# ziatdinovmax/pyroVED

Hardware: AMD Instinct MI355X
Metric: images/sec (SVI step) (higher is better)
Workload: dtype bf16; 1 GPU; C2 iVAE 28x28 invariances=['r','t'] latent_dim=2 bernoulli, batch 256 per GPU (global 256), bf16 MFMA operands for the hidden-layer contractions (fp32 accumulate; fp32 elsewhere); the guide (fc encoder, sample, split) runs in the decoder launch's prologue in fp32, SVI step = ELBO+grads+Adam; parallelism=dp1

## Files before the change

include/pyroved_amd.h:

```cpp
#ifndef PYROVED_AMD_H
#define PYROVED_AMD_H

#include <stdint.h>

#ifdef __cplusplus
extern "C" {
#endif

#define PV_ABI_VERSION 17

#define PV_EINVAL   (-1)
#define PV_EWS      (-2)
#define PV_ECOLL    (-3)

enum pv_act {
  PV_ACT_NONE = 0, PV_ACT_TANH = 1, PV_ACT_RELU = 2, PV_ACT_LRELU = 3,
  PV_ACT_SOFTPLUS = 4, PV_ACT_GELU = 5, PV_ACT_SIGMOID = 6
};

enum pv_lik { PV_LIK_BERNOULLI = 0, PV_LIK_GAUSSIAN = 1, PV_LIK_CBERNOULLI = 2 ,
  PV_LIK_POISSON_LOG = 3 };

enum pv_kl_mode { PV_KL_SAMPLED = 0, PV_KL_ANALYTIC = 1 };

// ... 87 lines not shown
  float   lr, adam_beta1, adam_beta2, adam_eps;
  int32_t adam_step;
  int32_t flags;
  void*   ev_start;
  void*   ev_stop;
  const float* class_onehot;
  void*   conv_ev_start;
  void*   conv_ev_stop;
  double* conv_ev_flops;
  int32_t dec_kernel;
  int32_t kl_mode;
} pv_ivae_plan;

int pv_version(void);
int pv_experiments_build(void);

#define PV_PLAN_ENC_TWO_LAUNCH 1
#define PV_PLAN_NO_SIDE_STREAM 2
#define PV_PLAN_ENC_NO_WAIT    4
#define PV_PLAN_NO_DEC1D       8
#define PV_PLAN_NO_ENC_FOLD    16
#define PV_PLAN_ENC_TILED      32
#define PV_PLAN_CONV_X3        64

int64_t pv_ivae_workspace_bytes(const pv_ivae_plan* plan);
#define PV_WS_ALL    0
#define PV_WS_STEP   1
#define PV_WS_ENCODE 2
#define PV_WS_DECODE 3
int64_t pv_ivae_workspace_bytes_for(const pv_ivae_plan* plan, int what);

int pv_ivae_uses_fused(const pv_ivae_plan* plan);

int pv_ivae_guide_folds(const pv_ivae_plan* plan);

int pv_ivae_loss_and_grads(const pv_ivae_plan* plan, int want_grads, void* stream);

int pv_adam_step(float* params, float* grads, float* m, float* v, int64_t n,
                 float lr, float beta1, float beta2, float eps, int32_t step, void* stream);

int pv_adam_step_hist(float* params, float* grads, float* m, float* v, int64_t n,
                      float lr, float beta1, float beta2, float eps, int32_t step,
                      const float* scalars_src, float* scalars_dst, int32_t n_scalars, void* stream);

int pv_ivae_guide(const pv_ivae_plan* plan, void* stream);
int pv_ivae_guide_backward(const pv_ivae_plan* plan, int want_grads, void* stream);
// ... 138 lines not shown
```

pyroved_amd/_abi.py:

```python
import contextlib
import ctypes as C
import functools
import os
import threading

import torch

PV_ABI_VERSION = 17
PV_PLAN_ENC_TWO_LAUNCH, PV_PLAN_NO_SIDE_STREAM, PV_PLAN_ENC_NO_WAIT, PV_PLAN_NO_DEC1D, PV_PLAN_NO_ENC_FOLD = 1, 2, 4, 8, 16
PV_PLAN_CONV_X3 = 64
PV_PLAN_ENC_TILED = 32
PV_MAX_LAYERS = 8

ACT = {None: 0, "none": 0, "tanh": 1, "relu": 2, "lrelu": 3, "softplus": 4, "gelu": 5, "sigmoid": 6}
LIK = {"bernoulli": 0, "gaussian": 1, "continuous_bernoulli": 2, "poisson_log": 3}
KL = {"sampled": 0, "analytic": 1}

_HERE = os.path.dirname(os.path.abspath(__file__))
LIB_PATH = os.environ.get("PV_LIB_PATH") or os.path.join(_HERE, "libpyroved_amd.so")
EXP_LIB_PATH = os.path.join(_HERE, "libpyroved_amd_exp.so")

c_float_p = C.POINTER(C.c_float)


class pv_layer(C.Structure):
    _fields_ = [("in_dim", C.c_int32), ("out_dim", C.c_int32), ("act", C.c_int32), ("_pad", C.c_int32),
                ("w_off", C.c_int64), ("b_off", C.c_int64)]


PV_MAX_OPS = 32
OP = {"conv": 1, "maxpool2": 2, "upsample2": 3, "upsample2_bilinear": 4, "batchnorm": 5}


class pv_op(C.Structure):
# ... 218 lines not shown
```

pyroved_amd/csrc/pv_plan.hip:

```cpp
#include "pv_common.h"
#include <algorithm>
#include <cmath>
#include <stdlib.h>
#include "pv_kernels.h"
#include "pv_sdec_fused.h"
#include "pv_linear.h"
#include "pv_convstack.h"
#include "pv_side.h"
#include "pv_conv.h"
#include "pv_particles.h"

namespace {

struct Carver {
  char* base;
  int64_t off;
  float* take(int64_t nfloats) {
    float* p = base ? (float*)(base + off) : nullptr;
    off += pv_align_up(nfloats * (int64_t)sizeof(float), 256);
    return p;
  }
};

struct Layout {
// ... 803 lines not shown
    if (L.renyi) pb.ll_s = L.llkb;
    if (st.chain) {
      pb.enc_n = p->n_enc; pb.enc_params = p->params; pb.enc_head = p->head;
      for (int i = 0; i < p->n_enc; ++i) { pb.enc_l[i] = p->enc[i]; pb.enc_act[i] = L.eact[i]; pb.enc_dp[i] = L.edp[i]; }
    }
  }
  st.wz = wgrad_problem(L.dhz, H, st.zin, st.ldz, p->grads + p->fc_latent.w_off, p->grads + p->fc_coord.b_off, S, lat_in, H);
  if (st.chain && f.part_rs && f.dhz_out && f.dzc_out && K == 0 && !p->row_w && p->kl_mode == PV_KL_SAMPLED && !p->row_elbo &&
      !p->dy && p->head.out_dim <= 16 && p->n_enc == 2 && p->enc[0].out_dim == FD_H && p->enc[1].in_dim == FD_H &&
      p->enc[1].out_dim == FD_H && p->head.in_dim == FD_H) {
    st.tail_np = one_launch_wgrad_problems(p, L, &st.wz, 1, st.tail);
    if (st.tail_np > 0 && adam) {
      auto lsz = [](const pv_layer& l) { return (int64_t)l.in_dim * l.out_dim + (l.b_off >= 0 ? l.out_dim : 0); };
      int64_t want = lsz(p->head) + lsz(p->fc_coord) + lsz(p->fc_latent) + lsz(p->out);
      for (int i = 0; i < p->n_enc; ++i) want += lsz(p->enc[i]);
      for (int i = 0; i < p->n_dec; ++i) want += lsz(p->dec[i]);
      int64_t cov = 2 * (int64_t)H * H + (int64_t)H * (3 + p->coord_dim) + 1;
      for (int i = 0; i < st.tail_np; ++i) cov += (int64_t)st.tail[i].M * st.tail[i].N + (st.tail[i].rowsumA ? st.tail[i].M : 0);
      if (cov != want || !adam_done || p->n_dec != 2) st.tail_np = -1;
    }
  }
  if (st.own_chain()) {
    PvEncFold& ef = st.ef;
    ef.chain = 1; ef.dhead = L.dhead; ef.ldh = (int)plan_head_w(p); ef.edp0 = L.edp[0]; ef.edp1 = L.edp[1]; ef.llb = L.llb;
  }
}

int fused_decoder_launch(FusedStep& st) {
  const pv_ivae_plan* p = st.p;
  const bool timed = p->ev_start && p->ev_stop;
  if (timed) (void)hipEventRecord((hipEvent_t)p->ev_start, st.s);
  if (p->fused >= 2) PV_TRY(pv_sdec_fused_bf16_launch(st.f, st.L.f_grid, st.grads, p->fused == 2, st.s, st.fold ? &st.ef : nullptr,
                                                      (st.own_chain() && !st.fold) ? &st.ef : nullptr));
  else PV_TRY(pv_sdec_fused_launch(st.f, st.L.f_grid, st.grads, st.s));
  if (timed) (void)hipEventRecord((hipEvent_t)p->ev_stop, st.s);
  return 0;
}

int fused_close_forward(const FusedStep& st) {
  const pv_ivae_plan* p = st.p; const Layout& L = st.L; hipStream_t s = st.s;
  const int64_t B = p->batch, N = p->n_pix, K = plan_K(p);
  if (K > 0) {
    PvLatentBwd lf{};
    lf.llrow = L.llrow; lf.llb = L.llb; lf.M = L.rows; lf.N = (int)N; lf.H = 0; lf.K = (int)K; lf.alpha = L.alpha;
    lf.hb.B = (int)B; lf.fwd_only = 1;
    PV_TRY(pv_latent_bwd(lf, s));
    return pv_finish_scalars(L.llb, (int)B, p->scalars, L.kl_part, L.kl_blocks, 1.0f, s);
// ... 552 lines not shown
```

pyroved_amd/csrc/pv_sdec_fused.h:

```cpp
#pragma once
#include "pv_common.h"

#define FD_H 128
#define FD_UNIT 16
#define FD_WAVES 8
#define FD_REC (2 * FD_H * FD_H + 14 * FD_H)
#define PV_RS_W 8
#define FB_WIMG_BYTES (4 * FD_H * FD_H * 2 + 256)

struct PvFused {
  const float* x;
  const float* grid;
  const float* tp;
  const float* hz;
  float hz_scale;
  const float *Wc, *bc;
  const float *W1, *b1;
  const float *W2, *b2;
  const float *wo, *bo;
  float* llrow;
  float* loc;
  float* rowtp;
  float* part_hz;
  float* part_rs;
// ... 10 lines not shown
  int64_t units;
  int N, cd, B, lik, sigmoid_out, kmax;
  int ablate;
  int qswap;
  float sig;
  int sel;
  int dl_exp;
};

struct PvEncFold {
  const float* params;
  pv_layer enc0, enc1, head;
  const float* x; int64_t ldx;
  const float* eps;
  float* eact0; float* eact1;
  float* head_out;
  float* z; float* z_scale; float* z_loc_out; float* z_scale_out;
  float* tp;
  float* kl_part;
  float* hz; const float* Wz;
  int lat_in, z_dim, coord_dim, has_r, has_t, has_s;
  float tp0, tp1, sc_prior, beta;
  int img_per_wg;
  int chain;
  float* dhead; int ldh;
  float* edp0; float* edp1;
  float* llb;
  int coop;
  unsigned* coop_flags;
};
#if defined(__HIP_DEVICE_COMPILE__)
typedef const __attribute__((address_space(4))) PvEncFold* PvEncFoldArg;
__device__ __forceinline__ PvEncFoldArg pv_kernarg_fold() {
  const __attribute__((address_space(4))) char* k = (const __attribute__((address_space(4))) char*)__builtin_amdgcn_kernarg_segment_ptr();
  PvEncFoldArg p = (PvEncFoldArg)(k + ((sizeof(PvFused) + alignof(PvEncFold) - 1) / alignof(PvEncFold)) * alignof(PvEncFold));
  asm volatile("" : "+s"(p));
  return p;
}
#else
typedef const PvEncFold* PvEncFoldArg;
__device__ inline PvEncFoldArg pv_kernarg_fold() { return nullptr; }
#endif
#define PV_GUIDE_IMG_MAX_BATCH 384
struct PvFbPrep;
bool pv_guide_img_ok(const PvEncFold& e, int B);
int pv_guide_img_launch(const PvEncFold& e, const PvFbPrep* prep, float hz_mul, int B, hipStream_t s, int kl_mode = PV_KL_SAMPLED);
// ... 152 lines not shown
```

pyroved_amd/csrc/pv_sdec_fused_w8.hip:

```cpp
#include "pv_sdec_fused.h"
#include "pv_fb_layout.h"
#include "pv_sdec_prims.h"
#include "pv_kernels.h"
#include <stdlib.h>

#define W8_WAVES 8
#define W8_ROWS (W8_WAVES * FD_UNIT)
#define W8_THREADS (64 * W8_WAVES)
#define W8_ARR (W8_ROWS * LDS2)
#define W8_ARR_BYTES (2 * W8_ARR)
#define WO_W1 0
#define WO_W2 IMG_BYTES
#define WO_SA (2 * IMG_BYTES)
#define WO_SB (WO_SA + W8_ARR_BYTES)
#define WO_VEC (WO_SB + W8_ARR_BYTES)
#define WO_ATAB (WO_VEC + 3 * FD_H * 4)
#define WO_TTAB (WO_ATAB + 8 * 64 * 8)
#define WO_INFO (WO_TTAB + 4 * 64 * 16)
#define WO_RED (WO_INFO + 3 * W8_ROWS * 4)
#define WO_CHZ (WO_RED + 256)
#define WO_CTP (WO_CHZ + W8_WAVES * FD_H * 4)
#define WO_CGR (WO_CTP + W8_WAVES * 256)
#define W8_LDS_BYTES (WO_CGR + W8_WAVES * 256)
#define WO_TX (WO_SB + 2 * 32 * LDS2)
// ... 6 lines not shown
#ifndef W8_FENCE_MASK
#define W8_FENCE_MASK 0
#endif
#define W8_FENCE() __builtin_amdgcn_sched_barrier(W8_FENCE_MASK)

__device__ __forceinline__ float w8_tanhc(float cx) {
  const float e = __builtin_amdgcn_exp2f(cx);
  return 1.0f - 2.0f * __builtin_amdgcn_rcpf(e + 1.0f);
}
#ifndef W8_HSWAP
#define W8_HSWAP 0
#endif
#ifndef W8_QSWAP
#define W8_QSWAP 1
#endif
bool pv_sdec_fused_w8_qswap() { return W8_QSWAP != 0; }
__device__ __forceinline__ bf16x8 w8_catq(const bf16x4& a, const bf16x4& b, int q) {
  return W8_QSWAP ? sd_catq(a, b, q >= 2) : sd_cat(a, b);
}
__device__ __forceinline__ float w8_sum_q(float v) {
  return pv_sum_rows(v);
}

#ifndef W8_ABL
#define W8_ABL 0
#endif
#ifndef W8_TAIL
#define W8_TAIL 1
#endif
#ifndef W8_OWN_SUMS
#define W8_OWN_SUMS 1
#endif
#define W8_ABL_LOADS(bit, g) (!(W8_ABL & (bit)) || (((g) & 1) == 0))
#define W8_ABL_BUF(bit, g) ((W8_ABL & (bit)) ? (((g) >> 1) & 1) : ((g) & 1))


struct W8Addr : SdAddr { int fs, hs; };
__device__ __forceinline__ W8Addr w8_addr(int r, int q) {
  W8Addr a;
  a.fs = W8_HSWAP ? ((r >> 2) & 1) : 0;
  a.hs = W8_HSWAP ? (q & 1) : (W8_QSWAP ? ((r >> 1) & 1) : 0);
  static_cast<SdAddr&>(a) = sd_addr(r, q);
  return a;
}

__device__ __forceinline__ void w8_layer_fwd(const __bf16* __restrict__ Wh, const float* __restrict__ bs,
// ... 103 lines not shown
#endif
  for (int ks = 0; ks < ksteps; ++ks) {
#if W8_ABL & 4
    if ((ks & 1) == 0) {
#else
    bf16x8 a[2], b[4];
    {
#endif
    a[0] = sd_cat(sd_tr_at(la0), sd_tr_at(la0 + ROW16));
    a[1] = sd_cat(sd_tr_at(la1), sd_tr_at(la1 + ROW16));
#pragma unroll
    for (int o = 0; o < 4; ++o) b[o] = sd_cat(sd_tr_at(lb + 32u * o), sd_tr_at(lb + 32u * o + ROW16));
    }
    W8_FENCE();
    accB = MFMA32(a[0], ones, accB);
#pragma unroll
    for (int o = 0; o < 4; ++o)
#pragma unroll
      for (int s_ = 0; s_ < 2; ++s_) accW[s_][o] = MFMA32(a[s_], b[o], accW[s_][o]);
    W8_FENCE();
    la0 += 2 * ROW16; la1 += 2 * ROW16; lb += 2 * ROW16;
  }
}

__device__ __forceinline__ void w8_colsum_mfma(__bf16* __restrict__ sc, const bf16x4 (&t)[8], const bf16x4& bop,
                                               f32x4 (&accS)[8], int wave, int r, int q) {
  sd_stage_store(sc, t, 16 * wave + r, q);
  sd_wait_lgkm0();
  const __bf16* base = sc + (16 * wave) * LDS2 + sd_stage_toff(r | sd_opaque0(), q);
  bf16x4 a[8];
#pragma unroll
  for (int jb = 0; jb < 8; ++jb) a[jb] = sd_tr(base + 16 * jb);
#pragma unroll
  for (int jb = 0; jb < 8; ++jb) accS[jb] = sd_mfma16(a[jb], bop, accS[jb]);
}

#ifdef W8_TRACE
__device__ long long w8_trace[512];
#define W8_STAMP(k)                                                                              \
  do {                                                                                           \
    if (g == 0 && lane == 0 && (wave == 0 || wave == 7) && tile_no < 8)                          \
      w8_trace[(wave ? 256 : 0) + tile_no * 16 + (k)] = (long long)__builtin_readcyclecounter(); \
  } while (0)
extern "C" int pv_debug_read_trace_w8(long long* out, int n) {
  if (n > 512) n = 512;
  return (int)hipMemcpyFromSymbol(out, HIP_SYMBOL(w8_trace), n * sizeof(long long));
// ... 62 lines not shown
  for (int i = 0; i < 4; ++i) h[i] = (__bf16)v[i];
  return h;
}
__device__ __forceinline__ f32x4 w8_mul_dtanh4(const f32x4& d, const bf16x4& hb) {
  const f32x4 t = sd_f32_of(hb);
  return d * (t * t - 1.0f);
}

#define WF_H1 WO_SA
#define WF_H2 (WF_H1 + 512)
#define WF_HD (WF_H2 + 512)
#define WF_P (WF_HD + 512)
#define WF_P_WAVE (64 * 17 * 4)
static_assert(WF_P + W8_WAVES * WF_P_WAVE <= WO_VEC, "guide scratch fits in the staging arrays");
#include "pv_gemv16.h"

#define W8_COOP_SPINS 4096
__device__ unsigned w8_coop_late_total;
extern "C" int pv_debug_coop_late_count(unsigned* out) {
  return (int)hipMemcpyFromSymbol(out, HIP_SYMBOL(w8_coop_late_total), sizeof(unsigned));
}
template <bool GRADS, int LIK, int FOLDK>
__global__ __launch_bounds__(W8_THREADS) void pv_sdec_w8_kernel(PvFused f, PvEncFold e) {
  constexpr bool FOLD = FOLDK != 0, CHAIN = FOLDK >= 2, COOP = FOLDK == 3;
  constexpr bool OWN = W8_OWN_SUMS && CHAIN && GRADS;
  extern __shared__ __attribute__((aligned(16))) char smb[];
  const int tid = threadIdx.x, lane0 = tid & 63, lane = lane0, r = lane & 15, q = lane >> 4;
  const int wave = __builtin_amdgcn_readfirstlane(tid >> 6);
  const int g = blockIdx.x, G = gridDim.x;
  const unsigned lds0 = __builtin_amdgcn_readfirstlane((unsigned)(size_t)smb);
  const __bf16* W1h = reinterpret_cast<const __bf16*>(smb + WO_W1);
  const __bf16* W2h = reinterpret_cast<const __bf16*>(smb + WO_W2);
  __bf16* sA = reinterpret_cast<__bf16*>(smb + WO_SA);
  __bf16* sB = reinterpret_cast<__bf16*>(smb + WO_SB);
  float* vec = reinterpret_cast<float*>(smb + WO_VEC);
  float* info = reinterpret_cast<float*>(smb + WO_INFO);
  float* red = reinterpret_cast<float*>(smb + WO_RED);
  const char* gimg = reinterpret_cast<const char*>(f.wimg);
  W8_STAMP_K(0);
  f32x4 xr[4], xpk;
  f32x4 xc[4][4];
  unsigned coop_tag = 0;
  if (COOP) {
    coop_tag = e.coop_flags[G] + 1u;
    const int K4 = (int)(e.ldx >> 2);
#pragma unroll
    for (int i = 0; i < 4; ++i) {
// ... 289 lines not shown
    __bf16* i1 = reinterpret_cast<__bf16*>(smb + WO_W1);
    __bf16* i2 = reinterpret_cast<__bf16*>(smb + WO_W2);
#pragma unroll
    for (int u = 0; u < 8; ++u) {
      const int idx = tid + W8_THREADS * u, row = idx >> 5, c4 = idx & 31;
      us4 h1, h2;
#pragma unroll
      for (int i = 0; i < 4; ++i) {
        h1[i] = __builtin_bit_cast(unsigned short, (__bf16)(w1v[u][i] * SD_C));
        h2[i] = __builtin_bit_cast(unsigned short, (__bf16)(w2v[u][i] * SD_C));
      }
      const int el = fb_wel(row, fb_pcol(4 * c4)) ^ (W8_HSWAP ? 4 * ((row >> 2) & 1) : 0) ^ (W8_QSWAP ? 4 * ((c4 >> 1) & 1) : 0);
      *reinterpret_cast<us4*>(i1 + el) = h1;
      *reinterpret_cast<us4*>(i2 + el) = h2;
    }
  }
  sd_wait_vm0();
  __syncthreads();
  W8_STAMP_K(1);
  const float bo = f.bo[0];
  typedef __attribute__((address_space(1))) float gfloat;
  unsigned long long u_llrow = 0, u_loc, u_rowtp = 0, u_part_hz = 0;
  int64_t a_M = 0;
  if constexpr (OWN) {
    asm volatile("s_mov_b64 %0, %1" : "=&s"(u_loc) : "s"((unsigned long long)f.loc));
  } else {
    asm volatile("s_mov_b64 %0, %5\n\ts_mov_b64 %1, %6\n\ts_mov_b64 %2, %7\n\ts_mov_b64 %3, %8\n\ts_mov_b64 %4, %9"
                 : "=&s"(u_llrow), "=&s"(u_loc), "=&s"(u_rowtp), "=&s"(u_part_hz), "=&s"(a_M)
                 : "s"((unsigned long long)f.llrow), "s"((unsigned long long)f.loc), "s"((unsigned long long)f.rowtp),
                   "s"((unsigned long long)f.part_hz), "s"(f.M));
  }
  gfloat* a_llrow = (gfloat*)u_llrow; gfloat* a_loc = (gfloat*)u_loc; gfloat* a_rowtp = (gfloat*)u_rowtp;
  gfloat* a_part_hz = (gfloat*)u_part_hz;

  f32x4 accW1[2][4], accW2[2][4], accS[8], accB1 = {0, 0, 0, 0}, accB2 = {0, 0, 0, 0};
#pragma unroll
  for (int kb = 0; kb < 8; ++kb) {
    accW1[kb >> 2][kb & 3] = f32x4{0, 0, 0, 0}; accW2[kb >> 2][kb & 3] = f32x4{0, 0, 0, 0}; accS[kb] = f32x4{0, 0, 0, 0};
  }
  float dbo = 0.0f;
  float llacc = 0.0f;
  int cur_b = -1;
  const int upb = f.N / FD_UNIT;
  float* rec = f.part + (int64_t)g * FD_REC;

  auto flush_hz = [&](int b) {
    const int64_t ub = (int64_t)b * upb;
    const int gfirst = (int)(((ub + 1) * G + f.units - 1) / f.units) - 1;
    gfloat* dst = a_part_hz + ((int64_t)b * f.kmax + (g - gfirst) * W8_WAVES + wave) * FD_H + 4 * q;
    if (r == 0) {
#pragma unroll
      for (int jb = 0; jb < 8; ++jb) *(__attribute__((address_space(1))) f32x4*)(dst + 16 * jb) = accS[jb] * SD_RC2;
    }
#pragma unroll
    for (int jb = 0; jb < 8; ++jb)
#pragma unroll
      for (int i = 0; i < 4; ++i) accS[jb][i] = r == 0 ? 0.0f : accS[jb][i];
  };

  const int u_lo = (int)((int64_t)g * f.units / G), u_hi = (int)((int64_t)(g + 1) * f.units / G);
  const int xun = (int)f.x_units;
  struct Pos { int unit, b, loc, xu; };
  auto pos_of = [&](int unit_) {
    Pos p_;
    p_.unit = unit_; p_.b = unit_ / upb; p_.loc = unit_ - p_.b * upb; p_.xu = xun > 0 ? unit_ % xun : unit_;
    return p_;
  };
  auto advance = [&](Pos& p_, int by) {
    p_.unit += by; p_.loc += by; p_.xu += by;
    while (p_.loc >= upb) { p_.loc -= upb; ++p_.b; }
    if (xun > 0) { while (p_.xu >= xun) p_.xu -= xun; }
  };
  const bool has_tail = W8_TAIL && ((u_hi - u_lo) & (W8_WAVES - 1)) == 1;
  const int u_end = has_tail ? u_hi - 1 : u_hi;
  const Pos pos_lo = pos_of(has_tail ? u_end : u_lo);
  Pos pos_cur = pos_of(u_lo + wave < u_end ? u_lo + wave : (has_tail ? u_end : u_lo));
  Pos pos_nx = pos_cur;
  float sw_next = 1.0f;
  auto x_of = [&](const Pos& p_) -> float {
    if (f.sw) sw_next = f.sw[p_.b];
    return f.x[(int64_t)p_.xu * FD_UNIT + r];
  };
  float xv_next = x_of(pos_cur);
  float* chz = reinterpret_cast<float*>(smb + WO_CHZ) + wave * FD_H;
  float* ctp = reinterpret_cast<float*>(smb + WO_CTP) + wave * 64;
  float* cgr = reinterpret_cast<float*>(smb + WO_CGR) + wave * 64;
  auto fetch_unit_inputs = [&](const Pos& p_, bool first) {
    const int n0 = p_.loc * FD_UNIT;
    if (!OWN || first) {
      sd_glds4(f.hz + (int64_t)p_.b * FD_H + lane, lds0 + WO_CHZ + wave * (FD_H * 4));
      sd_glds4(f.hz + (int64_t)p_.b * FD_H + 64 + lane, lds0 + WO_CHZ + wave * (FD_H * 4) + 256);
      sd_glds4(f.tp + (int64_t)p_.b * 8 + (lane & 7), lds0 + WO_CTP + wave * 256);
    }
    sd_glds4(f.grid + (int64_t)n0 * f.cd + (lane & (16 * f.cd - 1)), lds0 + WO_CGR + wave * 256);
  };
  fetch_unit_inputs(pos_cur, true);
  const W8Addr wad = w8_addr(r, q);
  int tile_no = -1;
  for (int ut = u_lo; ut < u_end; ut += W8_WAVES) {
    ++tile_no;
    (void)tile_no;
    asm volatile("; W8_TILE_BEGIN");
    W8_STAMP(0);
    const int nact = (u_end - ut) < W8_WAVES ? (u_end - ut) : W8_WAVES;
    if (ut + W8_WAVES + wave < u_end) advance(pos_nx, W8_WAVES);
    else pos_nx = pos_lo;
    int opq = 0;
    asm volatile("" : "+v"(opq));
    const int lane = lane0 | opq, r = lane & 15, q = lane >> 4;
    const float* wos = vec;
    const float* b1s = vec + FD_H;
    const float* b2s = vec + 2 * FD_H;
    const bool act = wave < nact;
    const int unit = act ? pos_cur.unit : ut;
    const int bu = pos_cur.b;
    const int64_t row = (int64_t)unit * FD_UNIT + r;
    float x0, x1, u0c, u1c, sc;
    sd_wait_vm0();
    {
      const float* t = ctp;
      const float* gr = cgr;
      if (f.cd == 2) {
        const float gx = gr[2 * r], gy = gr[2 * r + 1];
        u0c = gx * t[0] - gy * t[1];
        u1c = gx * t[1] + gy * t[0];
        sc = t[2];
        x0 = u0c * sc + t[3];
        x1 = u1c * sc + t[4];
      } else {
        u0c = gr[r]; u1c = 0.0f; sc = 1.0f;
        x0 = u0c + t[3]; x1 = 0.0f;
      }
    }
    const float xv = xv_next, swv = sw_next;
    float* inf_x0 = info + 16 * wave;
    float* inf_x1 = info + W8_ROWS + 16 * wave;
    float* inf_dl = info + 2 * W8_ROWS + 16 * wave;

    f32x4 tC[8];
    bf16x4 pA[8], h0b[8], h1b[8];
    float dlda = 0.0f;
    {
      bf16x4 bx = sd_zero4();
      {
        const float v = q == 0 ? x0 : x1;
        __bf16 vh, vl;
        fb_split(v, vh, vl);
        const __bf16 one = (__bf16)1.0f;
        if (q < 2) { bx[0] = vh; bx[1] = vl; bx[2] = vh; }
        else if (q == 2) { bx[0] = one; bx[1] = one; }
      }
      const bf16x4* atab = reinterpret_cast<const bf16x4*>(smb + WO_ATAB) + lane;
      const float* hzb = chz;
      bf16x4 aop[8];
#pragma unroll
      for (int jb = 0; jb < 8; ++jb) {
        tC[jb] = *reinterpret_cast<const f32x4*>(hzb + 16 * jb + 4 * q);
        aop[jb] = atab[64 * jb];
      }
      if (GRADS && q == 0) { inf_x0[r] = x0; inf_x1[r] = x1; }
      W8_FENCE();
      if (f.hz_scale == 0.0f) {
#pragma unroll
        for (int jb = 0; jb < 8; ++jb) tC[jb] = tC[jb] * SD_C;
      }
      W8_FENCE();
#pragma unroll
      for (int jb = 0; jb < 8; ++jb) tC[jb] = sd_mfma16(aop[jb], bx, tC[jb]);
      W8_FENCE();
      sd_tanh8<W8_FENCE_MASK>(tC);
      w8_cvt8(tC, h0b);
    }
    asm volatile("; W8_P1_coord_done");
    W8_STAMP(1);
    fetch_unit_inputs(pos_nx, false);
    {
      w8_layer_fwd(W1h, b1s, h0b, tC, wad, q);
      sd_tanh8<W8_FENCE_MASK>(tC);
      w8_cvt8(tC, h1b);
      asm volatile("; W8_P2_l1_done");
    W8_STAMP(2);
      w8_layer_fwd(W2h, b2s, h1b, tC, wad, q);
      sd_tanh8<W8_FENCE_MASK>(tC);
      f32x4 part4 = {0.0f, 0.0f, 0.0f, 0.0f};
#pragma unroll
      for (int jb = 0; jb < 8; ++jb) {
        const f32x4 wv = *reinterpret_cast<const f32x4*>(wos + 16 * jb + 4 * q);
        part4 = part4 + tC[jb] * wv;
        if (GRADS) {
#pragma unroll
          for (int i = 0; i < 4; ++i) pA[jb][i] = (__bf16)tC[jb][i];
          const f32x4 t2 = tC[jb] * tC[jb];
          tC[jb] = wv - wv * t2;
        }
      }
      const float a = w8_sum_q((part4[0] + part4[1]) + (part4[2] + part4[3])) + bo;
      float ll, locv;
      sd_pixel_lik<LIK>(a, xv, f.sig, f.sigmoid_out, ll, dlda, locv);
      dlda *= act ? swv : 0.0f;
      if (q == 0) {
        if (act) {
          if constexpr (OWN) llacc += ll;
          else if (a_llrow) a_llrow[row] = ll;
          if (a_loc) a_loc[row] = locv;
        }
        if (GRADS) { dbo += dlda; inf_dl[r] = dlda; }
      }
      xv_next = x_of(pos_nx);
    }
    pos_cur = pos_nx;
    asm volatile("; W8_P3_fwd_done");
    W8_STAMP(3);
    if (!GRADS) continue;
    const int ksteps = (nact + 1) >> 1;
    {
      sd_wait_lgkm0();
      const f32x4 d4 = *reinterpret_cast<const f32x4*>(inf_dl + 4 * q);
      bf16x4 bw = sd_zero4();
#pragma unroll
      for (int i = 0; i < 4; ++i) {
        __bf16 hi, lo;
        fb_split(d4[i], hi, lo);
        bw[i] = r == 3 ? hi : (r == 4 ? lo : (__bf16)0.0f);
      }
      w8_colsum_mfma(sA, pA, bw, accS, wave, r, q);
#pragma unroll
      for (int jb = 0; jb < 8; ++jb) tC[jb] = tC[jb] * dlda;
      w8_cvt8(tC, pA);
    }
    asm volatile("; W8_P4_dwo_done");
    W8_STAMP(4);
    sd_stage_store(sA, pA, 16 * wave + r, q);
    sd_stage_store(sB, h1b, 16 * wave + r, q);
    __syncthreads();
    asm volatile("; W8_P5_bar1");
    W8_STAMP(5);
    w8_wgrad_consume(sA, sB, accW2, accB2, wave, r, q, ksteps);
    asm volatile("; W8_P6_cons2");
    W8_STAMP(6);
    bf16x4 p0[8];
    {
      w8_layer_dgrad(W2h, pA, tC, wad);
      w8_mul_dtanh(tC, h1b);
      w8_cvt8(tC, pA);
      asm volatile("; W8_P7_dgrad2");
    W8_STAMP(7);
      w8_layer_dgrad(W1h, pA, tC, wad);
      w8_mul_dtanh(tC, h0b);
      w8_cvt8(tC, p0);
    }
    asm volatile("; W8_P8_dgrad1");
    W8_STAMP(8);
    __syncthreads();
    W8_STAMP(9);
    {
      if constexpr (!OWN) {
        f32x4 dd = {0.0f, 0.0f, 0.0f, 0.0f};
        const bf16x8* ttab = reinterpret_cast<const bf16x8*>(smb + WO_TTAB) + lane;
#pragma unroll
        for (int mm = 0; mm < 4; ++mm) dd = MFMA32(ttab[64 * mm], sd_cat(p0[2 * mm], p0[2 * mm + 1]), dd);
// ... 2 lines not shown
          a_rowtp[row] = sc * (d1 * u0c - d0 * u1c);
          a_rowtp[a_M + row] = d0 * u0c + d1 * u1c;
          a_rowtp[2 * a_M + row] = d0;
          a_rowtp[3 * a_M + row] = d1;
        }
        if (act && bu != cur_b) {
          if (cur_b >= 0) flush_hz(cur_b);
          cur_b = bu;
        }
      }
      const f32x4 a0 = *reinterpret_cast<const f32x4*>(inf_x0 + 4 * q);
      const f32x4 a1 = *reinterpret_cast<const f32x4*>(inf_x1 + 4 * q);
      bf16x4 bc_ = sd_zero4();
      const bool use1 = r == 2 || r == 6, lo_col = r >= 5;
#pragma unroll
      for (int i = 0; i < 4; ++i) {
        __bf16 hi, lo;
        fb_split(use1 ? a1[i] : a0[i], hi, lo);
        __bf16 v = lo_col ? lo : hi;
        if (r == 0) v = (__bf16)1.0f;
        if (r == 3 || r == 4 || r > 6) v = (__bf16)0.0f;
        bc_[i] = v;
      }
      w8_colsum_mfma(sA, p0, bc_, accS, wave, r, q);
      sd_wait_lgkm0();
    }
    asm volatile("; W8_P12_rowlocal");
    W8_STAMP(12);
    sd_stage_store(sA, pA, 16 * wave + r, q);
    sd_stage_store(sB, h0b, 16 * wave + r, q);
    __syncthreads();
    asm volatile("; W8_P10_bar3");
    W8_STAMP(10);
    w8_wgrad_consume(sA, sB, accW1, accB1, wave, r, q, ksteps);
    asm volatile("; W8_P11_cons1");
    W8_STAMP(11);
    __syncthreads();
    asm volatile("; W8_P13_bar4");
    W8_STAMP(13);
    W8_STAMP(14);
    asm volatile("; W8_TILE_END");
  }

  if (has_tail) {
    asm volatile("; W8_TAIL_BEGIN");
    const int lane = lane0, r = lane & 15, q = lane >> 4;
    const float* wos = vec;
    const float* b1s = vec + FD_H;
    const float* b2s = vec + 2 * FD_H;
    const int unit = u_end, bu = pos_cur.b;
    const int64_t row = (int64_t)unit * FD_UNIT + r;
    float x0, x1, u0c, u1c, sc;
    sd_wait_vm0();
    {
      const float* t = ctp;
      const float* gr = cgr;
      if (f.cd == 2) {
        const float gx = gr[2 * r], gy = gr[2 * r + 1];
        u0c = gx * t[0] - gy * t[1];
        u1c = gx * t[1] + gy * t[0];
        sc = t[2];
        x0 = u0c * sc + t[3];
        x1 = u1c * sc + t[4];
      } else {
        u0c = gr[r]; u1c = 0.0f; sc = 1.0f;
        x0 = u0c + t[3]; x1 = 0.0f;
      }
    }
    const float xv = xv_next, swv = sw_next;
// ... 417 lines not shown
      if (tid < FD_H) {
        float y = 0.0f;
#pragma unroll
        for (int jg = 0; jg < 16; ++jg) y += cs[256 + 128 * jg + tid];
        y *= pv_act_grad2(ch_a0, 0.0f, ep_->enc0.act);
        ep_->edp0[(int64_t)g * FD_H + tid] = y;
      }
    }
  }
  if (tid == 0) {
    float v = 0.0f;
    for (int w = 0; w < W8_WAVES; ++w) v += red[w];
    rec[2 * FD_H * FD_H + 5 * FD_H] = v;
  }
  W8_STAMP_K(3);
}

bool pv_sdec_fused_w8_fold_ok(const PvFused& f, int grid) {
  if (f.N % FD_UNIT != 0 || f.N > 1024 || f.N % 4 != 0 || grid < 1 || f.B % grid != 0 || f.x_units != 0) return false;
  const int ipw = f.B / grid;
  return ipw == 1 && f.units == (int64_t)f.B * (f.N / FD_UNIT);
}

int pv_sdec_fused_w8_launch(const PvFused& f_in, int grid, bool grads, hipStream_t s, const PvEncFold* fold) {
  PvFused f = f_in;
  static const int ablate = pv_exp_int("PV_FD_ABLATE", 0) & 1024;
  f.ablate = ablate;
  const size_t lds = W8_LDS_BYTES;
  const void* fn = nullptr;
  PvEncFold e{};
  if (fold) {
    if (!pv_sdec_fused_w8_fold_ok(f, grid)) return PV_EINVAL;
    e = *fold;
    e.img_per_wg = f.B / grid;
    if (e.coop && !(grid == 256 && e.enc0.out_dim == FD_H && e.coop_flags && e.chain)) e.coop = 0;
#ifndef PV_EXPERIMENTS
    e.coop = 0;
#endif
  }
#ifdef PV_EXPERIMENTS
#define W8_COOP_BUILD 3
#else
#define W8_COOP_BUILD 2
#endif
  const bool chain = fold && e.chain;
  if (chain && grads && !(f.part_rs && f.dhz_out && f.dzc_out)) return PV_EINVAL;
#define W8_PICK(G, L) fn = !fold ? reinterpret_cast<const void*>(&pv_sdec_w8_kernel<G, L, 0>)                     \
                               : (G && chain && e.coop) ? reinterpret_cast<const void*>(&pv_sdec_w8_kernel<G, L, G ? W8_COOP_BUILD : 1>) \
                               : (G && chain) ? reinterpret_cast<const void*>(&pv_sdec_w8_kernel<G, L, G ? 2 : 1>) \
                                                : reinterpret_cast<const void*>(&pv_sdec_w8_kernel<G, L, 1>)
  if (grads) {
    if (f.lik == PV_LIK_BERNOULLI) W8_PICK(true, PV_LIK_BERNOULLI);
    else if (f.lik == PV_LIK_GAUSSIAN) W8_PICK(true, PV_LIK_GAUSSIAN);
    else if (f.lik == PV_LIK_POISSON_LOG) W8_PICK(true, PV_LIK_POISSON_LOG);
    else W8_PICK(true, PV_LIK_CBERNOULLI);
  } else {
    if (f.lik == PV_LIK_BERNOULLI) W8_PICK(false, PV_LIK_BERNOULLI);
    else if (f.lik == PV_LIK_GAUSSIAN) W8_PICK(false, PV_LIK_GAUSSIAN);
    else if (f.lik == PV_LIK_POISSON_LOG) W8_PICK(false, PV_LIK_POISSON_LOG);
    else W8_PICK(false, PV_LIK_CBERNOULLI);
  }
#undef W8_PICK
  PV_TRY(pv_set_dynamic_lds(fn, (int)lds));
  void* args[] = {&f, &e};
  hipError_t e2 = hipLaunchKernel(fn, dim3(grid), dim3(W8_THREADS), args, lds, s);
  if (e2 != hipSuccess) return (int)e2;
  PV_LAUNCH_CHECK();
  return 0;
}
```

pyroved_amd/engine.py:

```python
import ctypes as C
import math
from typing import Dict, List, Optional

import torch
import torch.nn as nn

from . import _abi
from .nets.fc import fcEncoderNet, jfcEncoderNet, fcDecoderNet, sDecoderNet
from .nets.conv import convEncoderNet
from ._convplan import UnsupportedModel, conv_ops, fill_ops, bn_modules

ALIGN = 64
N_SCALARS = 4


def _kl_name(kl) -> str:
    if kl not in _abi.KL:
        raise ValueError("kl must be 'sampled' or 'analytic' (got %r)" % (kl,))
    return kl


def _particle_count(p) -> int:
    if isinstance(p, bool) or not isinstance(p, int) or p < 1:
        raise ValueError("particles must be an int >= 1 (got %r)" % (p,))
# ... 8 lines not shown
    a = float(a)
    if not math.isfinite(a) or a == 1.0:
        raise ValueError("renyi: alpha must be a finite float other than 1 (got %r); alpha -> 1 is the multi-particle ELBO, "
                         "which particles=P without renyi computes" % (a,))
    return a


def _linears(seq: nn.Sequential) -> List[nn.Linear]:
    return [m for m in seq if isinstance(m, nn.Linear)]


class IVAEEngine:
    supports_dp_step = True
    supports_scalars_out = True
    supports_step = True
    dec_kernel = 0
    enc_two_launch = False
    enc_no_wait = False
    side_stream = True
    dec1d = True
    enc_per_image = True
    conv_x3 = False
    enc_fold = True
    kl = "sampled"
    renyi = None

    def __init__(self, model, lr: float = 1e-3, betas=(0.9, 0.999), eps: float = 1e-8, fused: int = 2, kl: str = "sampled",
                 particles: int = 1, renyi=None):
        self.model = model
        self.kl = _kl_name(kl)
        self.particles = _particle_count(particles)
        self.renyi = _renyi_alpha(renyi)
        self.lr, self.betas, self.adam_eps = float(lr), (float(betas[0]), float(betas[1])), float(eps)
        self.fused = int(fused)
        self.adam_t = 0
        self.grads_live = False
        self.device = None
        self.flat = self.grad = self.m = self.v = None
        self.ws = None
        self.events = (None, None)
        self._bn_enc, self._bn_dec = [], []
        self._enc_opt = None
        self._enc_params = []
        self._layout: Dict[str, int] = {}
        self._views: Dict[str, torch.Tensor] = {}
        self._check_model()
# ... 274 lines not shown
        if not self._conv_slices or self.wide_weights:
            return
        self._conv_tick += 1
        if not force and self._conv_tick % self._CONV_W_EVERY != 1:
            return
        if torch.cuda.is_current_stream_capturing():
            self._conv_tick -= 1
            return
        mx = float(torch.stack([self.flat[o:o + n].abs().max() for o, n in self._conv_slices]).max())
        if mx >= self._CONV_W_HI or 0.0 < mx < self._CONV_W_LO or mx != mx:
            import warnings
            warnings.warn("pyroved_amd: a convolution weight reached |w| = %.3g, outside the range of the fp16-piece "
                          "kernels; this model switches to the range-free bf16-piece convolution kernels (three pieces at "
                          "fp32-class precision, the two-piece mixed form at the throughput precision)" % mx)
            self.wide_weights = True

    def _plan_flags(self) -> int:
        return ((_abi.PV_PLAN_ENC_TWO_LAUNCH if getattr(self, "enc_two_launch", False) else 0) |
                (0 if getattr(self, "side_stream", True) else _abi.PV_PLAN_NO_SIDE_STREAM) |
                (_abi.PV_PLAN_ENC_NO_WAIT if getattr(self, "enc_no_wait", False) else 0) |
                (0 if getattr(self, "dec1d", True) else _abi.PV_PLAN_NO_DEC1D) |
                (0 if getattr(self, "enc_fold", True) else _abi.PV_PLAN_NO_ENC_FOLD) |
                (0 if getattr(self, "enc_per_image", True) else _abi.PV_PLAN_ENC_TILED) |
                (_abi.PV_PLAN_CONV_X3 if getattr(self, "conv_x3", False) else 0))

    def ensure_bound(self):
        if not self._bound():
            self.bind()

    def _layer(self, prefix: str, lin: nn.Linear, act) -> _abi.pv_layer:
        l = _abi.pv_layer()
        l.in_dim, l.out_dim, l.act = lin.in_features, lin.out_features, _abi.ACT[act]
        l.w_off = self._layout[prefix + ".weight"]
        l.b_off = self._layout[prefix + ".bias"] if lin.bias is not None else -1
        return l

    def _fc_encoder_plan(self, p, enc, m):
        idx = [i for i, mod in enumerate(enc.fc_layers) if isinstance(mod, nn.Linear)]
        p.n_enc = len(idx)
        for j, i in enumerate(idx):
            p.enc[j] = self._layer("encoder_z.fc_layers.%d" % i, enc.fc_layers[i], enc.activation)
        h = _abi.pv_layer()
        h.in_dim, h.out_dim, h.act = enc.fc11.in_features, 2 * m.z_dim + self.K, 0
        h.w_off, h.b_off = self._layout["encoder_z.fc11.weight"], self._layout["encoder_z.fc11.bias"]
        assert self._layout["encoder_z.fc12.weight"] == h.w_off + enc.fc11.weight.numel()
        assert self._layout["encoder_z.fc12.bias"] == h.b_off + enc.fc11.bias.numel()
# ... 405 lines not shown
```

Before: 2.781 million images/s.

## Add specialized full-tile decoder loop for image-owning fused training kernel

Adds a FOLDK==4 template build of the fused w8 decoder kernel used when each workgroup owns one image whose unit count is a multiple of the wave count (plus an optional tail). Applicable configurations are ones with no sample weights, 2-D coordinates, a nonzero hz scale and a non-Gaussian likelihood. This build drops per-tile position bookkeeping, partial-tile masking and runtime branches, and uses compile-time-unrolled weight-gradient consumes. It also prefetches the grid straight into LDS with global_load_lds and precomputes the staging offsets once per tile. The cost is another kernel instantiation (more code and compile time), and a plan flag is added to fall back to the generic loop.

```diff
diff --git a/include/pyroved_amd.h b/include/pyroved_amd.h
--- a/include/pyroved_amd.h
+++ b/include/pyroved_amd.h
@@ -133,6 +133,7 @@
 #define PV_PLAN_NO_ENC_FOLD    16
 #define PV_PLAN_ENC_TILED      32
 #define PV_PLAN_CONV_X3        64
+#define PV_PLAN_GENERIC_TILE_LOOP 128
 
 int64_t pv_ivae_workspace_bytes(const pv_ivae_plan* plan);
 #define PV_WS_ALL    0
diff --git a/pyroved_amd/_abi.py b/pyroved_amd/_abi.py
--- a/pyroved_amd/_abi.py
+++ b/pyroved_amd/_abi.py
@@ -10,6 +10,7 @@
 PV_PLAN_ENC_TWO_LAUNCH, PV_PLAN_NO_SIDE_STREAM, PV_PLAN_ENC_NO_WAIT, PV_PLAN_NO_DEC1D, PV_PLAN_NO_ENC_FOLD = 1, 2, 4, 8, 16
 PV_PLAN_CONV_X3 = 64
 PV_PLAN_ENC_TILED = 32
+PV_PLAN_GENERIC_TILE_LOOP = 128
 PV_MAX_LAYERS = 8
 
 ACT = {None: 0, "none": 0, "tanh": 1, "relu": 2, "lrelu": 3, "softplus": 4, "gelu": 5, "sigmoid": 6}
diff --git a/pyroved_amd/csrc/pv_plan.hip b/pyroved_amd/csrc/pv_plan.hip
--- a/pyroved_amd/csrc/pv_plan.hip
+++ b/pyroved_amd/csrc/pv_plan.hip
@@ -849,7 +849,8 @@
   }
   if (st.own_chain()) {
     PvEncFold& ef = st.ef;
-    ef.chain = 1; ef.dhead = L.dhead; ef.ldh = (int)plan_head_w(p); ef.edp0 = L.edp[0]; ef.edp1 = L.edp[1]; ef.llb = L.llb;
+    ef.chain = 1 | ((p->flags & PV_PLAN_GENERIC_TILE_LOOP) ? PV_CHAIN_GENERIC_LOOP : 0);
+    ef.dhead = L.dhead; ef.ldh = (int)plan_head_w(p); ef.edp0 = L.edp[0]; ef.edp1 = L.edp[1]; ef.llb = L.llb;
   }
 }
 
diff --git a/pyroved_amd/csrc/pv_sdec_fused.h b/pyroved_amd/csrc/pv_sdec_fused.h
--- a/pyroved_amd/csrc/pv_sdec_fused.h
+++ b/pyroved_amd/csrc/pv_sdec_fused.h
@@ -56,6 +56,7 @@
   int lat_in, z_dim, coord_dim, has_r, has_t, has_s;
   float tp0, tp1, sc_prior, beta;
   int img_per_wg;
+#define PV_CHAIN_GENERIC_LOOP 2
   int chain;
   float* dhead; int ldh;
   float* edp0; float* edp1;
diff --git a/pyroved_amd/csrc/pv_sdec_fused_w8.hip b/pyroved_amd/csrc/pv_sdec_fused_w8.hip
--- a/pyroved_amd/csrc/pv_sdec_fused_w8.hip
+++ b/pyroved_amd/csrc/pv_sdec_fused_w8.hip
@@ -52,6 +52,12 @@
   return pv_sum_rows(v);
 }
 
+__device__ __forceinline__ void w8_glds4_s(const __attribute__((address_space(1))) void* sbase, unsigned voff, unsigned lds_dst) {
+  unsigned keep;
+  asm volatile("s_mov_b32 %0, m0\n\ts_mov_b32 m0, %3\n\ts_nop 0\n\tglobal_load_lds_dword %1, %2\n\ts_mov_b32 m0, %0"
+               : "=&s"(keep) : "v"(voff), "s"(sbase), "s"(lds_dst) : "memory");
+}
+
 #ifndef W8_ABL
 #define W8_ABL 0
 #endif
@@ -201,6 +207,59 @@
     la0 += 2 * ROW16; la1 += 2 * ROW16; lb += 2 * ROW16;
   }
 }
+struct W8Stage { int se, to; };
+__device__ __forceinline__ W8Stage w8_stage_offs(int wave, int r, int q) {
+  r |= sd_opaque0();
+  W8Stage s;
+  s.se = (16 * wave + r) * LDS2 + 4 * (q ^ ((r >> 2) & 3));
+  s.to = sd_stage_toff(r, q);
+  return s;
+}
+__device__ __forceinline__ void w8_stage_store_at(__bf16* __restrict__ sh, const bf16x4 (&h)[8], int se) {
+#pragma unroll
+  for (int jb = 0; jb < 8; ++jb) *reinterpret_cast<bf16x4*>(sh + se + 16 * jb) = h[jb];
+}
+__device__ __forceinline__ void w8_colsum_mfma_at(__bf16* __restrict__ sc, const bf16x4 (&t)[8], const bf16x4& bop, f32x4 (&accS)[8],
+                                                  int wave, const W8Stage& st) {
+  w8_stage_store_at(sc, t, st.se);
+  sd_wait_lgkm0();
+  const __bf16* base = sc + (16 * wave) * LDS2 + st.to;
+  bf16x4 a[8];
+#pragma unroll
+  for (int jb = 0; jb < 8; ++jb) a[jb] = sd_tr(base + 16 * jb);
+#pragma unroll
+  for (int jb = 0; jb < 8; ++jb) accS[jb] = sd_mfma16(a[jb], bop, accS[jb]);
+}
+template <int KS>
+__device__ __forceinline__ void w8_wgrad_consume_k(const __bf16* sa, const __bf16* sb, f32x4 (&accW)[2][4], f32x4& accB,
+                                                   int wave, int toff) {
+  const int jp = wave >> 1, kh = wave & 1;
+  const short one = 0x3f80;
+  const short8_ ones_s = {one, one, one, one, one, one, one, one};
+  const bf16x8 ones = __builtin_bit_cast(bf16x8, ones_s);
+  unsigned la0 = (unsigned)(size_t)sa + 2u * (unsigned)(toff + 32 * jp + 16 * kh);
+  unsigned la1 = (unsigned)(size_t)sa + 2u * (unsigned)(toff + 32 * jp + 16 * (1 ^ kh));
+  unsigned lb = (unsigned)(size_t)sb + 2u * (unsigned)(toff + 64 * kh);
+  asm volatile("" : "+v"(la0), "+v"(la1), "+v"(lb));
+  constexpr unsigned ROW16 = 2u * 16 * LDS2;
+  static_assert((2 * KS - 1) * ROW16 + 96 + 8 <= 65535, "every read of the unrolled consume is base + immediate");
+#pragma unroll
+  for (int ks = 0; ks < KS; ++ks) {
+    const unsigned k0 = 2u * ROW16 * ks;
+    bf16x8 a[2], b[4];
+    a[0] = sd_cat(sd_tr_at(la0 + k0), sd_tr_at(la0 + k0 + ROW16));
+    a[1] = sd_cat(sd_tr_at(la1 + k0), sd_tr_at(la1 + k0 + ROW16));
+#pragma unroll
+    for (int o = 0; o < 4; ++o) b[o] = sd_cat(sd_tr_at(lb + k0 + 32u * o), sd_tr_at(lb + k0 + 32u * o + ROW16));
+    W8_FENCE();
+    accB = MFMA32(a[0], ones, accB);
+#pragma unroll
+    for (int o = 0; o < 4; ++o)
+#pragma unroll
+      for (int s_ = 0; s_ < 2; ++s_) accW[s_][o] = MFMA32(a[s_], b[o], accW[s_][o]);
+    W8_FENCE();
+  }
+}
 
 __device__ __forceinline__ void w8_colsum_mfma(__bf16* __restrict__ sc, const bf16x4 (&t)[8], const bf16x4& bop,
                                                f32x4 (&accS)[8], int wave, int r, int q) {
@@ -309,7 +368,8 @@
 }
 template <bool GRADS, int LIK, int FOLDK>
 __global__ __launch_bounds__(W8_THREADS) void pv_sdec_w8_kernel(PvFused f, PvEncFold e) {
-  constexpr bool FOLD = FOLDK != 0, CHAIN = FOLDK >= 2, COOP = FOLDK == 3;
+  constexpr bool FOLD = FOLDK != 0, CHAIN = FOLDK >= 2, COOP = FOLDK == 3, FULL = FOLDK == 4;
+  static_assert(!FULL || (GRADS && W8_OWN_SUMS && W8_TAIL), "the full-tile loop is the image-owning training build's");
   constexpr bool OWN = W8_OWN_SUMS && CHAIN && GRADS;
   extern __shared__ __attribute__((aligned(16))) char smb[];
   const int tid = threadIdx.x, lane0 = tid & 63, lane = lane0, r = lane & 15, q = lane >> 4;
@@ -645,7 +705,13 @@
   typedef __attribute__((address_space(1))) float gfloat;
   unsigned long long u_llrow = 0, u_loc, u_rowtp = 0, u_part_hz = 0;
   int64_t a_M = 0;
-  if constexpr (OWN) {
+  unsigned long long u_x = 0, u_grid = 0;
+  if constexpr (FULL) {
+    const int64_t r0 = (int64_t)g * f.N;
+    asm volatile("s_mov_b64 %0, %3\n\ts_mov_b64 %1, %4\n\ts_mov_b64 %2, %5"
+                 : "=&s"(u_loc), "=&s"(u_x), "=&s"(u_grid)
+                 : "s"((unsigned long long)(f.loc ? f.loc + r0 : nullptr)), "s"((unsigned long long)(f.x + r0)), "s"((unsigned long long)f.grid));
+  } else if constexpr (OWN) {
     asm volatile("s_mov_b64 %0, %1" : "=&s"(u_loc) : "s"((unsigned long long)f.loc));
   } else {
     asm volatile("s_mov_b64 %0, %5\n\ts_mov_b64 %1, %6\n\ts_mov_b64 %2, %7\n\ts_mov_b64 %3, %8\n\ts_mov_b64 %4, %9"
@@ -681,7 +747,7 @@
       for (int i = 0; i < 4; ++i) accS[jb][i] = r == 0 ? 0.0f : accS[jb][i];
   };
 
-  const int u_lo = (int)((int64_t)g * f.units / G), u_hi = (int)((int64_t)(g + 1) * f.units / G);
+  const int u_lo = FULL ? 0 : (int)((int64_t)g * f.units / G), u_hi = FULL ? upb : (int)((int64_t)(g + 1) * f.units / G);
   const int xun = (int)f.x_units;
   struct Pos { int unit, b, loc, xu; };
   auto pos_of = [&](int unit_) {
@@ -697,14 +763,16 @@
   const bool has_tail = W8_TAIL && ((u_hi - u_lo) & (W8_WAVES - 1)) == 1;
   const int u_end = has_tail ? u_hi - 1 : u_hi;
   const Pos pos_lo = pos_of(has_tail ? u_end : u_lo);
-  Pos pos_cur = pos_of(u_lo + wave < u_end ? u_lo + wave : (has_tail ? u_end : u_lo));
+  Pos pos_cur = FULL ? Pos{wave, g, wave, g * upb + wave} : pos_of(u_lo + wave < u_end ? u_lo + wave : (has_tail ? u_end : u_lo));
   Pos pos_nx = pos_cur;
   float sw_next = 1.0f;
   auto x_of = [&](const Pos& p_) -> float {
     if (f.sw) sw_next = f.sw[p_.b];
     return f.x[(int64_t)p_.xu * FD_UNIT + r];
   };
-  float xv_next = x_of(pos_cur);
+  float xv_next = 0.0f;
+  if constexpr (FULL) xv_next = ((const gfloat*)u_x + wave * FD_UNIT)[r];
+  else xv_next = x_of(pos_cur);
   float* chz = reinterpret_cast<float*>(smb + WO_CHZ) + wave * FD_H;
   float* ctp = reinterpret_cast<float*>(smb + WO_CTP) + wave * 64;
   float* cgr = reinterpret_cast<float*>(smb + WO_CGR) + wave * 64;
@@ -725,17 +793,22 @@
     (void)tile_no;
     asm volatile("; W8_TILE_BEGIN");
     W8_STAMP(0);
-    const int nact = (u_end - ut) < W8_WAVES ? (u_end - ut) : W8_WAVES;
-    if (ut + W8_WAVES + wave < u_end) advance(pos_nx, W8_WAVES);
-    else pos_nx = pos_lo;
+    const int nact = FULL ? W8_WAVES : ((u_end - ut) < W8_WAVES ? (u_end - ut) : W8_WAVES);
+    int unit_nx = 0;
+    if constexpr (FULL) {
+      unit_nx = ut + W8_WAVES < u_end ? ut + W8_WAVES + wave : (has_tail ? u_end : 0);
+    } else {
+      if (ut + W8_WAVES + wave < u_end) advance(pos_nx, W8_WAVES);
+      else pos_nx = pos_lo;
+    }
     int opq = 0;
     asm volatile("" : "+v"(opq));
     const int lane = lane0 | opq, r = lane & 15, q = lane >> 4;
     const float* wos = vec;
     const float* b1s = vec + FD_H;
     const float* b2s = vec + 2 * FD_H;
-    const bool act = wave < nact;
-    const int unit = act ? pos_cur.unit : ut;
+    const bool act = FULL || wave < nact;
+    const int unit = FULL ? ut + wave : (act ? pos_cur.unit : ut);
     const int bu = pos_cur.b;
     const int64_t row = (int64_t)unit * FD_UNIT + r;
     float x0, x1, u0c, u1c, sc;
@@ -743,7 +816,7 @@
     {
       const float* t = ctp;
       const float* gr = cgr;
-      if (f.cd == 2) {
+      if (FULL || f.cd == 2) {
         const float gx = gr[2 * r], gy = gr[2 * r + 1];
         u0c = gx * t[0] - gy * t[1];
         u1c = gx * t[1] + gy * t[0];
@@ -783,7 +856,7 @@
       }
       if (GRADS && q == 0) { inf_x0[r] = x0; inf_x1[r] = x1; }
       W8_FENCE();
-      if (f.hz_scale == 0.0f) {
+      if (!FULL && f.hz_scale == 0.0f) {
 #pragma unroll
         for (int jb = 0; jb < 8; ++jb) tC[jb] = tC[jb] * SD_C;
       }
@@ -796,7 +869,8 @@
     }
     asm volatile("; W8_P1_coord_done");
     W8_STAMP(1);
-    fetch_unit_inputs(pos_nx, false);
+    if constexpr (FULL) w8_glds4_s((const gfloat*)u_grid + unit_nx * (2 * FD_UNIT), 4u * (unsigned)(lane & 31), lds0 + WO_CGR + wave * 256);
+    else fetch_unit_inputs(pos_nx, false);
     {
       w8_layer_fwd(W1h, b1s, h0b, tC, wad, q);
       sd_tanh8<W8_FENCE_MASK>(tC);
@@ -820,22 +894,27 @@
       const float a = w8_sum_q((part4[0] + part4[1]) + (part4[2] + part4[3])) + bo;
       float ll, locv;
       sd_pixel_lik<LIK>(a, xv, f.sig, f.sigmoid_out, ll, dlda, locv);
-      dlda *= act ? swv : 0.0f;
+      if constexpr (!FULL) dlda *= act ? swv : 0.0f;
       if (q == 0) {
-        if (act) {
+        if constexpr (FULL) {
+          llacc += ll;
+          if (a_loc) (a_loc + unit * FD_UNIT)[r] = locv;
+        } else if (act) {
           if constexpr (OWN) llacc += ll;
           else if (a_llrow) a_llrow[row] = ll;
           if (a_loc) a_loc[row] = locv;
         }
         if (GRADS) { dbo += dlda; inf_dl[r] = dlda; }
       }
-      xv_next = x_of(pos_nx);
-    }
-    pos_cur = pos_nx;
+      if constexpr (FULL) xv_next = ((const gfloat*)u_x + unit_nx * FD_UNIT)[r];
+      else xv_next = x_of(pos_nx);
+    }
+    if constexpr (!FULL) pos_cur = pos_nx;
     asm volatile("; W8_P3_fwd_done");
     W8_STAMP(3);
     if (!GRADS) continue;
     const int ksteps = (nact + 1) >> 1;
+    W8Stage stg{};
     {
       sd_wait_lgkm0();
       const f32x4 d4 = *reinterpret_cast<const f32x4*>(inf_dl + 4 * q);
@@ -846,19 +925,21 @@
         fb_split(d4[i], hi, lo);
         bw[i] = r == 3 ? hi : (r == 4 ? lo : (__bf16)0.0f);
       }
-      w8_colsum_mfma(sA, pA, bw, accS, wave, r, q);
+      if constexpr (FULL) { stg = w8_stage_offs(wave, r, q); w8_colsum_mfma_at(sA, pA, bw, accS, wave, stg); }
+      else w8_colsum_mfma(sA, pA, bw, accS, wave, r, q);
 #pragma unroll
       for (int jb = 0; jb < 8; ++jb) tC[jb] = tC[jb] * dlda;
       w8_cvt8(tC, pA);
     }
     asm volatile("; W8_P4_dwo_done");
     W8_STAMP(4);
-    sd_stage_store(sA, pA, 16 * wave + r, q);
-    sd_stage_store(sB, h1b, 16 * wave + r, q);
+    if constexpr (FULL) { w8_stage_store_at(sA, pA, stg.se); w8_stage_store_at(sB, h1b, stg.se); }
+    else { sd_stage_store(sA, pA, 16 * wave + r, q); sd_stage_store(sB, h1b, 16 * wave + r, q); }
     __syncthreads();
     asm volatile("; W8_P5_bar1");
     W8_STAMP(5);
-    w8_wgrad_consume(sA, sB, accW2, accB2, wave, r, q, ksteps);
+    if constexpr (FULL) w8_wgrad_consume_k<W8_WAVES / 2>(sA, sB, accW2, accB2, wave, stg.to);
+    else w8_wgrad_consume(sA, sB, accW2, accB2, wave, r, q, ksteps);
     asm volatile("; W8_P6_cons2");
     W8_STAMP(6);
     bf16x4 p0[8];
@@ -907,17 +988,19 @@
         if (r == 3 || r == 4 || r > 6) v = (__bf16)0.0f;
         bc_[i] = v;
       }
-      w8_colsum_mfma(sA, p0, bc_, accS, wave, r, q);
+      if constexpr (FULL) { stg = w8_stage_offs(wave, r, q); w8_colsum_mfma_at(sA, p0, bc_, accS, wave, stg); }
+      else w8_colsum_mfma(sA, p0, bc_, accS, wave, r, q);
       sd_wait_lgkm0();
     }
     asm volatile("; W8_P12_rowlocal");
     W8_STAMP(12);
-    sd_stage_store(sA, pA, 16 * wave + r, q);
-    sd_stage_store(sB, h0b, 16 * wave + r, q);
+    if constexpr (FULL) { w8_stage_store_at(sA, pA, stg.se); w8_stage_store_at(sB, h0b, stg.se); }
+    else { sd_stage_store(sA, pA, 16 * wave + r, q); sd_stage_store(sB, h0b, 16 * wave + r, q); }
     __syncthreads();
     asm volatile("; W8_P10_bar3");
     W8_STAMP(10);
-    w8_wgrad_consume(sA, sB, accW1, accB1, wave, r, q, ksteps);
+    if constexpr (FULL) w8_wgrad_consume_k<W8_WAVES / 2>(sA, sB, accW1, accB1, wave, stg.to);
+    else w8_wgrad_consume(sA, sB, accW1, accB1, wave, r, q, ksteps);
     asm volatile("; W8_P11_cons1");
     W8_STAMP(11);
     __syncthreads();
@@ -929,7 +1012,7 @@
 
   if (has_tail) {
     asm volatile("; W8_TAIL_BEGIN");
-    const int lane = lane0, r = lane & 15, q = lane >> 4;
+    const int lane = FULL ? (lane0 | sd_opaque0()) : lane0, r = lane & 15, q = lane >> 4;
     const float* wos = vec;
     const float* b1s = vec + FD_H;
     const float* b2s = vec + 2 * FD_H;
@@ -1393,6 +1476,15 @@
   return ipw == 1 && f.units == (int64_t)f.B * (f.N / FD_UNIT);
 }
 
+#define W8_FULL_BUILD (W8_OWN_SUMS && W8_TAIL && !(W8_ABL & 4))
+static bool w8_full_tile_ok(const PvFused& f, int grid) {
+  const int upb = f.N / FD_UNIT;
+  return W8_FULL_BUILD && pv_sdec_fused_w8_fold_ok(f, grid) && upb >= W8_WAVES && (upb & (W8_WAVES - 1)) <= 1 && !f.sw && f.cd == 2 &&
+         f.hz_scale != 0.0f && f.lik != PV_LIK_GAUSSIAN;
+}
+static int w8_last_fold_build = -1;
+extern "C" int pv_debug_w8_last_fold_build(void) { return __atomic_load_n(&w8_last_fold_build, __ATOMIC_RELAXED); }
+
 int pv_sdec_fused_w8_launch(const PvFused& f_in, int grid, bool grads, hipStream_t s, const PvEncFold* fold) {
   PvFused f = f_in;
   static const int ablate = pv_exp_int("PV_FD_ABLATE", 0) & 1024;
@@ -1416,8 +1508,17 @@
 #endif
   const bool chain = fold && e.chain;
   if (chain && grads && !(f.part_rs && f.dhz_out && f.dzc_out)) return PV_EINVAL;
+  const bool full = chain && grads && !e.coop && !(e.chain & PV_CHAIN_GENERIC_LOOP) && w8_full_tile_ok(f, grid);
+#if W8_FULL_BUILD
+#define W8_FULL_ID 4
+#else
+#define W8_FULL_ID 2
+#endif
+  const int build = !fold ? 0 : (grads && chain) ? (e.coop ? W8_COOP_BUILD : (full ? W8_FULL_ID : 2)) : 1;
+  if (fold) __atomic_store_n(&w8_last_fold_build, build, __ATOMIC_RELAXED);
 #define W8_PICK(G, L) fn = !fold ? reinterpret_cast<const void*>(&pv_sdec_w8_kernel<G, L, 0>)                     \
                                : (G && chain && e.coop) ? reinterpret_cast<const void*>(&pv_sdec_w8_kernel<G, L, G ? W8_COOP_BUILD : 1>) \
+                               : (G && full) ? reinterpret_cast<const void*>(&pv_sdec_w8_kernel<G, L, G ? ((L) == PV_LIK_GAUSSIAN ? 2 : W8_FULL_ID) : 1>) \
                                : (G && chain) ? reinterpret_cast<const void*>(&pv_sdec_w8_kernel<G, L, G ? 2 : 1>) \
                                                 : reinterpret_cast<const void*>(&pv_sdec_w8_kernel<G, L, 1>)
   if (grads) {
diff --git a/pyroved_amd/engine.py b/pyroved_amd/engine.py
--- a/pyroved_amd/engine.py
+++ b/pyroved_amd/engine.py
@@ -54,6 +54,7 @@
     enc_per_image = True
     conv_x3 = False
     enc_fold = True
+    full_tile_loop = True
     kl = "sampled"
     renyi = None
 
@@ -374,6 +375,7 @@
                 (0 if getattr(self, "dec1d", True) else _abi.PV_PLAN_NO_DEC1D) |
                 (0 if getattr(self, "enc_fold", True) else _abi.PV_PLAN_NO_ENC_FOLD) |
                 (0 if getattr(self, "enc_per_image", True) else _abi.PV_PLAN_ENC_TILED) |
+                (0 if getattr(self, "full_tile_loop", True) else _abi.PV_PLAN_GENERIC_TILE_LOOP) |
                 (_abi.PV_PLAN_CONV_X3 if getattr(self, "conv_x3", False) else 0))
 
     def ensure_bound(self):
```

Result: faster. 2.845 million images/s, median of 6 (+2.3%).
